# robotic-vision-lab/Edge-Informed-Contrast-Maximization

Hardware: AMD Instinct MI355X
Metric: warped-events/sec/GPU + loss+grad eval ms, 1e6 events @ 346x260 (higher is better)
Workload: dtype f32

## Files before the change

edge-informed-contrast-maximization_amd/csrc/eincm_api.hip:

```cpp
#include <hip/hip_runtime.h>
#include <hip/hip_ext.h>

#include <algorithm>
#include <chrono>
#include <cmath>
#include <cstdarg>
#include <cstdio>
#include <cstdlib>
#include <cstring>
#include <string>
#include <vector>

#include "eincm.h"
#include "eincm_kernels.hip.h"
#include "eincm_kernels_f64.hip.h"
#include "eincm_binning.hip.h"
#include "eincm_edges.hip.h"
#include "eincm_objectives.hip.h"
#include "eincm_splat_window.hip.h"
#include "eincm_canny.hip.h"
#include "eincm_preprocess.hip.h"
#include "eincm_gtflow.hip.h"
#include "eincm_dsec.hip.h"
#include "eincm_floweval.hip.h"
// ... 39 lines not shown
        if (p) { v.push_back(Block{p, bytes}); total += bytes; }
        return hipSuccess;
    }
    static bool drop(std::vector<Block>& v, size_t& total, void* p, hipError_t (*free_fn)(void*)) {
        for (size_t i = 0; i < v.size(); ++i)
            if (v[i].p == p) { (void)free_fn(p); total -= v[i].bytes; v.erase(v.begin() + i); return true; }
        return false;
    }
};

template <typename T, bool PINNED = false> struct Grow {
    T* p = nullptr;
    size_t n = 0;
};

struct Carve {
    size_t total = 0;
    size_t add(size_t bytes) { const size_t off = total; total += (bytes + 255) & ~(size_t)255; return off; }
};

struct SegList {
    int seg = 0;
    int n = 0;
    double tspan = 1.0;
    Item* d_items = nullptr;
    int32_t* d_order = nullptr;
    std::vector<Item> h_items;
    std::vector<int32_t> h_order;
    int32_t* d_win_item0 = nullptr;
    std::vector<int32_t> h_win_item0;
    Window* d_wins = nullptr;
    int32_t* d_itembase = nullptr;
    unsigned grid(int R) const { return (unsigned)(((n + NXCD - 1) / NXCD) * NXCD * R); }
};

struct WinFit {
    int cap, maxw;
    bool pal;
    bool fits;
};

struct EvalPlan {
    enum Shape { IDENTITY, TWO_DOF, GRID } shape = GRID;
    enum ThetaSrc { THETA_DEVICE, THETA_ARGS, THETA_PINNED, THETA_PIECES } theta_src = THETA_PIECES;
    int h = 0, w = 0; size_t nth = 0;
    bool want_grad = false, full_aux = false, div_grad = false;
    EvalParams ep{};
    bool obj = false; ObjGeom og{};
    int wincap = 0, winmaxw = 0, pitch_aligned = 0, wincap_a = 0, winmaxw_a = 0;
    WinFit win_2{}; bool splat_short = false;
    bool use_arg = false, use_arg_big = false;
    bool need_theta_image = false;
    bool host_asm = false;
    bool grid_tail = false;
    bool stream_stats = false, g2_from_imgrad = false;
    bool tv_proj = false, proj = false;
    bool all_r = false;
    bool events_projected = false; int nsrc = 0;
    bool zero_copy_out = false;
};

struct StagePlan {
    Geom g{};
    int64_t N = 0;
    int seg = 0, seg_s = 0, seg_2 = 0;
    bool splat_short = false;
    int pitch = 0;
    bool sort_segments = true;
    bool spread = true;
    bool host_binning = false;
    bool defer_constants = false;
    bool wide = false;
};

constexpr int SEG_SHORT = 8192;
constexpr int MIN_SEG = 64;

struct StageArgs {
    int B, R; const int64_t* n_events;
    const int16_t* const* xs; const int16_t* const* ys; const double* const* ts; const double* const* edges; const double* edge_ts;
    uint32_t flags;
};

struct StageScratch {
    std::vector<unsigned> cntmax; std::vector<double> dtmax;
    bool edge_ts_uploaded = false;
    std::vector<BinBlock> blks; std::vector<int32_t> win_blk; int32_t misc[4]; std::vector<double> mom;
    std::vector<uint32_t> sxy; std::vector<double> st; std::vector<float> ef;
    std::vector<int> ishift;
};

}

struct eincm_ctx {
    int device = 0;
    int H = 0, W = 0, maxR = 0, maxB = 0;
    int64_t maxN = 0;
    uint32_t cflags = 0;
    int seg = 0;
    int seg_s = 0;
    hipStream_t stream = nullptr;
    std::string err;
    Mem mem;

    bool staged = false;
    StagePlan stage;
    Geom g{};
    std::vector<int64_t> win_events;

    uint32_t* d_xy = nullptr;
    double* d_t = nullptr;
    uint32_t* d_xy_g = nullptr;
    double* d_t_g = nullptr;
    std::vector<int32_t> h_tilecount;
    SegList gather;
    SegList splat;
    SegList splat_sh;
    SegList gather_2;
    bool policy_evaluated = false;
    int wincap = WIN_CAP_DEFAULT;
    bool wincap_fixed = false;
    int16_t* d_raw_x = nullptr; int16_t* d_raw_y = nullptr; double* d_raw_t = nullptr;
    BinBlock* d_binblocks = nullptr; int32_t* d_win_blk = nullptr; uint32_t* d_blockhist = nullptr;
    int32_t* d_tilecount = nullptr; int32_t* d_tilebase = nullptr; int32_t* d_bin_misc = nullptr;
    bool itembase_valid = false;
    double* d_edges_raw = nullptr; double* d_edge_moments = nullptr;
    int64_t max_binblocks = 0;
    bool host_binning = false;
    int64_t max_items = 0;
    float* d_edges = nullptr;
    double* d_edge_ts = nullptr;
    unsigned long long* d_acc = nullptr;
    float* d_iwe = nullptr;
    float* d_G = nullptr;
    float* d_zero_iwe = nullptr;
    double* d_Theta = nullptr;
    double* d_theta_in = nullptr;
    long long* d_gTheta = nullptr;
    double* d_g11 = nullptr;
    double* d_dtmax = nullptr;
    unsigned* d_gmax = nullptr;
// ... 304 lines not shown
            tr[(size_t)ty * tilesX + tx] = q;
        }
    HIPCHK(c, hipMemcpyAsync(c->d_tilerng, tr.data(), tr.size() * sizeof(TileRange), hipMemcpyHostToDevice, c->stream));
    c->proj_in_gather = fits && !getenv("EINCM_NO_PROJ_IN_GATHER");
    HIPCHK(c, hipStreamSynchronize(c->stream));
    c->cur_h = h; c->cur_w = w; c->cur_method = method;
    return EINCM_OK;
}

constexpr size_t ZERO_COPY_MAX = 65536;


int win_maxw(int cap) { return std::max(40, (int)std::lround(std::sqrt((double)cap * 1.4))); }

WinFit fit_window(double vmax, double tspan, double margin, int floor_k, int pitch) {
    static const int caps[] = {2304, 3072, 4608, 6912};
    const double side = TS + margin + vmax * tspan, sd = std::ceil(side);
    const double need = pitch < 0 ? side * side : sd * sd;
    int cap = caps[3];
    for (int k = floor_k; k < 4; ++k) if (need <= caps[k]) { cap = caps[k]; break; }
    return WinFit{cap, win_maxw(cap), pitch > 0 && std::ceil(sd / 32.0) * 32.0 * sd <= (double)cap, need <= (double)caps[3]};
}

int clear_accumulators(eincm_ctx* c) {
    const size_t img = (size_t)c->H * c->W;
    HIPCHK(c, hipMemsetAsync(c->d_acc, 0, (size_t)c->maxB * c->maxR * img * sizeof(unsigned long long), c->stream));
    HIPCHK(c, hipMemsetAsync(c->d_gTheta, 0, (size_t)c->maxB * img * 2 * sizeof(long long), c->stream));
    HIPCHK(c, hipMemsetAsync(c->d_gth.p, 0, (size_t)2 * c->maxB * c->coarse_cap * sizeof(long long), c->stream));
    c->acc_dirty = false;
    return EINCM_OK;
}

void launch_theta_image(eincm_ctx* c, int h, int w, bool identity, bool use_arg, const ThetaArgBig& targ, const double* theta_dev,
                        bool with_windows) {
    const Geom& g = c->g;
    const bool ww = with_windows && c->itembase_valid;
    auto go = [&](auto kernel, const auto& ta) {
        launch_timed(c, EINCM_STAGE_THETA, kernel, dim3(g.ntiles, g.B), dim3(NT), 0, g, h, w, identity ? 1 : 0, use_arg ? 1 : 0, ta,
                     theta_dev, c->d_AH.p, c->d_AW.p, c->d_rowtap, c->d_coltap, c->d_tilerng, c->d_Theta, c->d_tmm, c->d_edge_ts,
                     c->gather.n, c->gather.d_items, ww ? c->gather.d_itembase : nullptr, c->gather.d_wins,
                     c->splat.n, c->splat.d_items, ww ? c->splat.d_itembase : nullptr, c->splat.d_wins);
    };
    if (!use_arg || (size_t)g.B * h * w * 2 <= (size_t)THETA_ARG_MID) {
        ThetaArgMid mid;
        if (use_arg) memcpy(mid.v, targ.v, (size_t)g.B * h * w * 2 * sizeof(double));
        go(k_theta<ThetaArgMid>, mid);
// ... 31 lines not shown
    {
        StageTimer t(c, EINCM_STAGE_THETA, two_dof ? !P.need_theta_image : c->itembase_valid);
        const SegList &ga = c->gather, &sp = c->splat;
        const int nwin_threads = (ga.n + sp.n) * g.R;
        if (two_dof) {
            if (theta_host) c->last_theta11.assign(theta_host, theta_host + (size_t)g.B * 2); else c->last_theta11.clear();
            c->Theta_valid = false;
            if (P.need_theta_image) launch_theta_image(c, P.h, P.w, false, P.use_arg_big, targ_big, theta_dev, false);
            if (!P.host_asm)
                launch_timed(c, EINCM_STAGE_THETA, k_theta_const, dim3((std::max(g.B * g.ntiles, nwin_threads) + NT - 1) / NT), dim3(NT), 0, g,
                                   P.use_arg ? 1 : 0, targ, theta_dev, c->d_tmm, c->d_edge_ts, ga.n, ga.d_items, ga.d_wins,
                                   sp.n, sp.d_items, sp.d_wins);
        } else {
            launch_theta_image(c, P.h, P.w, P.shape == EvalPlan::IDENTITY, P.use_arg_big, targ_big, theta_dev, true);
            if (nwin_threads > 0 && !c->itembase_valid)
                hipLaunchKernelGGL(k_windows, dim3((nwin_threads + NT - 1) / NT), dim3(NT), 0, c->stream, g, c->d_tmm, c->d_edge_ts,
                                   ga.n, ga.d_items, ga.d_wins, sp.n, sp.d_items, sp.d_wins);
        }
    }
    {
        StageTimer t(c, EINCM_STAGE_SPLAT, true);
        c->acc_dirty = true;
        if (c->splat.n > 0) {
            const SegList& L = P.splat_short ? c->splat_sh : c->splat;
            const size_t theta_tile = two_dof ? 0 : TS * TS * sizeof(double2);
            const int use_arg = P.use_arg ? 1 : 0;
            if (c->splat_rad != 1) {
                Geom gs = g;
                gs.wincap = std::min(g.wincap, two_dof ? SW_CAP_CONST : SW_CAP_TILE);
                gs.winmaxw = win_maxw(gs.wincap);
                auto go = [&](auto kernel) {
                    launch_timed(c, EINCM_STAGE_SPLAT, kernel, dim3(L.grid(g.R)), dim3(NT), (size_t)gs.wincap * sizeof(unsigned long long) + theta_tile,
                                 gs, L.n, L.d_items, c->d_xy, c->d_t, c->d_Theta, c->d_tmm, c->d_edge_ts, c->d_acc, L.d_order, use_arg, theta_dev, targ);
                };
                if (two_dof) c->splat_rad == 0 ? go(k_splat_r<THETA_CONST, 0>) : c->splat_rad == 2 ? go(k_splat_r<THETA_CONST, 2>) : go(k_splat_r<THETA_CONST, 3>);
                else         c->splat_rad == 0 ? go(k_splat_r<THETA_TILE, 0>) : c->splat_rad == 2 ? go(k_splat_r<THETA_TILE, 2>) : go(k_splat_r<THETA_TILE, 3>);
            } else {
                auto go = [&](auto kernel) {
                    launch_timed(c, EINCM_STAGE_SPLAT, kernel, dim3(L.grid(g.R)), dim3(512), (size_t)g.wincap * sizeof(float) + theta_tile, g, L.n,
                                 L.d_items, c->d_xy, c->d_t, c->d_Theta, c->d_edge_ts, c->splat.d_wins, c->d_acc, L.d_order, use_arg, theta_dev, targ);
                };
                two_dof ? go(k_splat<THETA_CONST, 512>) : go(k_splat<THETA_TILE, 512>);
            }
        }
    }
    HIPCHK(c, hipGetLastError());
    c->pend.theta_dev = theta_dev; c->pend.targ = targ;
// ... 232 lines not shown
    if (c->fp64) return P;
    const size_t nall = (size_t)g.B * P.nth;

    static const bool no_big_arg = getenv("EINCM_NO_BIG_THETA_ARG") != nullptr;
    P.use_arg = !c->theta_dev_in && !identity && nall <= (size_t)THETA_ARG_MAX;
    P.use_arg_big = !c->theta_dev_in && !identity && nall <= (size_t)THETA_ARG_BIG && !no_big_arg;
    P.theta_src = c->theta_dev_in ? EvalPlan::THETA_DEVICE
                : (P.use_arg_big && (P.use_arg || !two_dof)) ? EvalPlan::THETA_ARGS
                : nall <= ZERO_COPY_MAX ? EvalPlan::THETA_PINNED : EvalPlan::THETA_PIECES;
    P.need_theta_image = !two_dof || ep.want_tv || c->theta_dev_in;

    P.wincap = g.wincap; P.winmaxw = g.winmaxw; P.wincap_a = g.wincap_a; P.winmaxw_a = g.winmaxw_a;
    P.pitch_aligned = c->stage.pitch != 0 ? 1 : 0;
    P.win_2 = WinFit{c->wincap, win_maxw(c->wincap), c->stage.pitch >= 2, true};
    if (!c->wincap_fixed) {
        double vmax = 0.0;
        const size_t stride = nall > 8192 ? nall / 8192 : 1;
        if (c->theta_dev_in) vmax = (c->vmax_hint >= 0.0 && std::isfinite(c->vmax_hint)) ? c->vmax_hint : 1e9;
        else if (stride == 1) { for (size_t i = 0; i < nall; ++i) { const double a = std::fabs(theta_host[i]); vmax = std::max(vmax, a <= 1.7e308 ? a : 0.0); } }
        else for (size_t i = 0; i < nall; i += stride) { const double a = std::fabs(theta_host[i]); if (a > vmax && std::isfinite(a)) vmax = a; }
        const double margin = 2.0 * (c->splat_rad + 1);
        const int floor_s = two_dof ? 2 : 0, pitch_s = c->stage.pitch != 0 ? 1 : 0;
        WinFit s = fit_window(vmax, c->splat.tspan, margin, floor_s, pitch_s);
        P.splat_short = two_dof && c->splat_sh.n > 0 && !s.fits;
        if (P.splat_short) s = fit_window(vmax, c->splat_sh.tspan, margin, floor_s, pitch_s);
        P.wincap = s.cap; P.winmaxw = s.maxw; P.pitch_aligned = s.pal ? 1 : 0;
        const WinFit a = fit_window(vmax, c->gather.tspan, margin, 2, -1);
        P.wincap_a = a.cap; P.winmaxw_a = a.maxw;
        P.win_2 = fit_window(vmax, c->gather_2.tspan, margin, 2, c->stage.pitch >= 2 ? 1 : 0);
    }

    static const bool no_host_asm = getenv("EINCM_NO_HOST_ASM") != nullptr;
    const bool tail_ok = c->splat_rad == 1 && P.shape == EvalPlan::GRID && c->proj_in_gather && c->itembase_valid && nall <= ZERO_COPY_MAX &&
                         !c->theta_dev_in;
    P.host_asm = want_grad && ((two_dof && !ep.want_tv) || tail_ok) && !ep.want_div && !P.full_aux && !no_host_asm && !c->device_results &&
                 !c->theta_dev_in;
    P.grid_tail = P.host_asm && P.shape == EvalPlan::GRID;
    P.g2_from_imgrad = want_grad && ep.contrast_kind == EINCM_CONTRAST_GRAD_MAG && !P.obj;
    P.stream_stats = P.host_asm || (P.g2_from_imgrad && g.ntiles >= NSPART) || P.obj;
    P.tv_proj = ep.use_tv_grad && P.shape == EvalPlan::GRID && c->proj_in_gather;
    P.proj = want_grad && P.shape == EvalPlan::GRID && c->proj_in_gather && c->splat_rad == 1;
    static const int all_r_env = getenv("EINCM_GATHER_ALL_R") ? atoi(getenv("EINCM_GATHER_ALL_R")) : -1;
    P.all_r = P.proj && (all_r_env >= 0 ? all_r_env != 0 : c->gather.n >= 700);
    P.events_projected = two_dof || P.proj;
    P.nsrc = (!want_grad || identity) ? 0 : (P.events_projected ? 0 : 1) + ((ep.use_tv_grad && !P.tv_proj) ? 1 : 0);
    P.zero_copy_out = !c->device_results && !c->theta_dev_in && !identity && nall <= ZERO_COPY_MAX;
    return P;
}

void scan_theta(eincm_ctx* c, const double* theta_host, size_t nth) {
    c->theta_nan.assign((size_t)c->g.B, 0);
    for (int b = 0; b < c->g.B; ++b) {
// ... 147 lines not shown
                           c->d_wc, c->d_objc.p, c->d_gdiv.p, c->d_dgparts.p, c->d_G, c->d_gmax, c->h_ovals.p, 0);
    }
    if (want_grad) {
        {
            StageTimer t(c, EINCM_STAGE_IMGRAD, !P.div_grad && !P.obj);
            if (P.div_grad)
                hipLaunchKernelGGL(k_divgrad, dim3(g.ntiles, g.R, g.B), dim3(NT), 0, c->stream, g, c->d_iwe, c->d_parts,
                                   c->d_gdiv.p, c->d_dgparts.p);
            if (P.obj) {
                const ObjGeom& og = P.og;
                hipLaunchKernelGGL(k_obj_parts, dim3(og.ncells, g.R, g.B), dim3(NT), 0, c->stream, g, og, c->d_iwe, 1, c->d_edges, c->d_oparts.p);
                hipLaunchKernelGGL(k_obj_grad, dim3(n_imwg, g.R, g.B), dim3(IG_NT), 0, c->stream, g, ep, og, c->d_iwe, c->d_edges, c->d_oparts.p,
                                   c->d_wc, c->d_objc.p, c->d_gdiv.p, c->d_dgparts.p, c->d_G, c->d_gmax, c->h_ovals.p, 1);
            } else {
                launch_timed(c, EINCM_STAGE_IMGRAD, k_imgrad, dim3(n_imwg, g.R, g.B), dim3(IG_NT), 0, g, ep, c->d_iwe, c->d_edges,
                                   c->d_parts, c->d_wc, c->d_gdiv.p, c->d_dgparts.p, host_asm ? c->h_g2 : c->d_g2parts, c->d_G, c->d_gmax,
                                   host_asm ? c->h_img : nullptr, host_asm ? 1 : 0);
            }
        }
        {
            StageTimer t(c, EINCM_STAGE_GATHER, true);
            constexpr int NT_TILE = 512;
            if (c->gather.n > 0) {
                const SegList& L = two_dof ? c->gather_2 : c->gather;
                const uint32_t* xy_g = two_dof ? c->d_xy : c->d_xy_g;
                const double* t_g = two_dof ? c->d_t : c->d_t_g;
                Geom gg = g;
                if (two_dof) { gg.pitch_aligned = P.win_2.pal ? 1 : 0; gg.wincap_a = P.win_2.cap; gg.winmaxw_a = P.win_2.maxw; }
                const dim3 grid(L.grid(P.all_r ? 1 : g.R));
                const size_t lds = gg.wincap_a * sizeof(float) + (two_dof ? 0 : TS * TS * 2 * sizeof(double) + TS * TS * sizeof(double2));
                double* g11 = host_asm ? c->h_g11 : c->d_g11;
                const int use_arg = P.use_arg ? 1 : 0;
                if (c->splat_rad != 1) {
                    auto go = [&](auto kernel) {
                        launch_timed(c, EINCM_STAGE_GATHER, kernel, grid, dim3(NT), lds, gg, L.n, L.d_items, xy_g, t_g, c->d_Theta, c->d_tmm,
                                     c->d_edge_ts, c->d_G, c->d_gTheta, g11, c->d_wc, c->d_gmax, c->stage.wide ? 1 : 0, use_arg, c->pend.theta_dev,
                                     c->pend.targ);
                    };
                    if (two_dof) c->splat_rad == 0 ? go(k_gather_r<THETA_CONST, 0>) : c->splat_rad == 2 ? go(k_gather_r<THETA_CONST, 2>) : go(k_gather_r<THETA_CONST, 3>);
                    else         c->splat_rad == 0 ? go(k_gather_r<THETA_TILE, 0>) : c->splat_rad == 2 ? go(k_gather_r<THETA_TILE, 2>) : go(k_gather_r<THETA_TILE, 3>);
                } else {
                    auto go = [&](auto kernel, int nthreads) {
                        launch_timed(c, EINCM_STAGE_GATHER, kernel, grid, dim3(nthreads), lds, gg, L.n, L.d_items, xy_g, t_g, c->d_Theta,
                                     c->d_edge_ts, c->d_G, c->gather.d_wins, c->d_gTheta, g11, c->d_wc, c->d_gmax, L.d_order, use_arg,
                                     c->pend.theta_dev, c->pend.targ, P.h, P.w, c->d_AH.p, c->d_AW.p, c->d_tilerng, c->d_gth.p, (int)c->coarse_cap,
                                     P.grid_tail ? 1 : 0, c->d_gticket, c->gather.d_win_item0, c->h_grad,
                                     (P.grid_tail && ep.use_tv_grad) ? ep.gamma : 0.0, c->d_tvparts, c->d_gth.p + (size_t)c->maxB * c->coarse_cap);
                    };
                    if (two_dof)      go(k_gather<THETA_CONST, 0, NT, 0>, NT);
                    else if (P.all_r) c->stage.wide ? go(k_gather<THETA_TILE, 1, NT_TILE, 1, 1>, NT_TILE) : go(k_gather<THETA_TILE, 0, NT_TILE, 1, 1>, NT_TILE);
                    else if (c->stage.wide) P.proj ? go(k_gather<THETA_TILE, 1, NT_TILE, 1>, NT_TILE) : go(k_gather<THETA_TILE, 1, NT_TILE, 0>, NT_TILE);
                    else              P.proj ? go(k_gather<THETA_TILE, 0, NT_TILE, 1>, NT_TILE) : go(k_gather<THETA_TILE, 0, NT_TILE, 0>, NT_TILE);
                }
            }
        }
        if (P.nsrc > 0) {
            StageTimer t(c, EINCM_STAGE_PROJECT, true);
            launch_timed(c, EINCM_STAGE_PROJECT, k_project, dim3(g.ntiles, g.B, P.nsrc), dim3(NT), 0, g, P.h, P.w,
                               (int)c->coarse_cap, P.events_projected ? 1 : 0, c->stage.wide ? 1 : 0, c->d_AH.p, c->d_AW.p, c->d_rowtap, c->d_coltap, c->d_gTheta, c->d_tvg,
                               c->d_wc, c->d_gmax, c->d_gth.p, c->d_gth.p + (size_t)c->maxB * c->coarse_cap);
        }
    }
    if (!host_asm) {
        StageTimer t(c, EINCM_STAGE_FINAL, !(want_grad && identity));
        launch_timed(c, EINCM_STAGE_FINAL, k_final, dim3(g.B), dim3(FT), 0, g, ep, c->d_parts, c->d_divparts, c->d_tvparts,
                           c->d_tmm, c->d_wc, P.g2_from_imgrad ? c->d_g2parts : nullptr, c->d_gth.p, c->d_gth.p + (size_t)c->maxB * c->coarse_cap, (int)c->coarse_cap,
                           c->d_g11, c->gather_2.d_win_item0, c->gather_2.n, c->d_gmax,
                           P.zero_copy_out ? c->h_outs : c->d_outs, P.zero_copy_out ? c->h_grad : c->d_grad, want_grad ? 1 : 0);
        if (want_grad && identity) {
            hipLaunchKernelGGL(k_final_dense, dim3(256, g.B), dim3(NT), 0, c->stream, g, ep.use_tv_grad, c->stage.wide ? 1 : 0, c->d_gTheta,
                               c->d_tvg, c->d_wc, c->d_gmax, c->d_outs, c->d_grad);
        }
    }
    HIPCHK(c, hipGetLastError());
    c->n_pieces = 0;
    c->pend.copy_mode = (P.zero_copy_out || host_asm) ? 0 : 1;
    if (c->pend.copy_mode && !c->device_results) { const int rcc = enqueue_result_copies(c); if (rcc) return rcc; c->pend.copy_mode = 0; }
    if (timing && c->ring_size == 1) { (void)hipEventRecord(c->ev[c->ring_cur][EINCM_N_STAGES][1], c->stream); c->ev_used[c->ring_cur][EINCM_N_STAGES] = true; }
    c->pend.launched = true;
    c->acc_dirty = false;
    return EINCM_OK;
}

void host_assemble(eincm_ctx* c) {
    const Geom& g = c->g;
    const EvalPlan& P = c->pend.plan;
    const EvalParams& ep = P.ep;
    const double HW = (double)g.H * (double)g.W;
    for (int b = 0; b < g.B; ++b) {
        const WinConst& wc = c->h_wc[b];
// ... 1 lines not shown
        memset(&o, 0, sizeof o);
        if (b < 64 && !((g.wmask >> b) & 1ull)) continue;
        double sum_rel_con = 0.0, sum_rel_corr = 0.0;
        for (int r = 0; r < g.R; ++r) {
            const double* q = c->h_img + ((size_t)b * g.R + r) * IMGSCAL_N;
            ImgScal s{};
            s.m = q[0]; s.M = q[1]; s.D = q[2]; s.cm = q[3]; s.cM = q[4]; s.sI = q[5]; s.sII = q[6]; s.sEI = q[7];
            double g2 = 0.0;
            const int nwg = (g.nig + IG_NT / 64 - 1) / (IG_NT / 64);
            const double* g2p = c->h_g2 + ((size_t)b * g.R + r) * nwg;
            for (int i = 0; i < nwg; ++i) g2 += g2p[i];
            const double mse = mse_from_moments(s, wc.sE[r], wc.sEE[r], HW);
            const double mean = s.sI / HW;
            const double var = s.sII / HW - mean * mean;
            const double cgm = g2 / HW;
            const double con = (ep.contrast_kind == 1) ? var : cgm;
            const double c0 = (ep.contrast_kind == 1) ? wc.c0_var : wc.c0_gradmag;
            o.corr[r] = -mse; o.contrast_gm[r] = cgm; o.var[r] = var; o.div[r] = NAN;
            sum_rel_con += wc.mrw[r] * con / (c0 + EPSN);
            sum_rel_corr += wc.mrw[r] * (-mse) / (wc.zc[r] + EPSN);
        }
        assemble_window(ep, g.R, sum_rel_con, sum_rel_corr, NAN, window_tv(c, ep, b), c->theta_nan[b] != 0, true, o);
        if (P.shape == EvalPlan::TWO_DOF) {
            const int lo = c->gather_2.h_win_item0[b], hi = c->gather_2.h_win_item0[b + 1];
            const double* p = c->h_g11 + (size_t)lo * g.R * 2;
            const size_t n = (size_t)(hi - lo) * g.R;
            double ax[4] = {0.0, 0.0, 0.0, 0.0}, ay[4] = {0.0, 0.0, 0.0, 0.0};
            size_t k = 0;
            for (; k + 4 <= n; k += 4) {
                ax[0] += p[2 * k]; ay[0] += p[2 * k + 1]; ax[1] += p[2 * k + 2]; ay[1] += p[2 * k + 3];
                ax[2] += p[2 * k + 4]; ay[2] += p[2 * k + 5]; ax[3] += p[2 * k + 6]; ay[3] += p[2 * k + 7];
            }
            for (; k < n; ++k) { ax[0] += p[2 * k]; ay[0] += p[2 * k + 1]; }
            c->h_grad[(size_t)b * 2] = (ax[0] + ax[1]) + (ax[2] + ax[3]); c->h_grad[(size_t)b * 2 + 1] = (ay[0] + ay[1]) + (ay[2] + ay[3]);
        } else if (c->win_events[b] == 0) {
            for (size_t i = 0; i < P.nth; ++i) c->h_grad[(size_t)b * P.nth + i] = 0.0;
        }
    }
}

int eval_end_collect(eincm_ctx* c, double* value, double* grad, eincm_aux* aux) {
    if (!c->pend.active || !c->pend.launched) return fail(c, EINCM_ERR_STATE, "no evaluation in flight");
    const Geom& g = c->g;
    const bool want_grad = c->pend.plan.want_grad;
    const size_t nth = c->pend.plan.nth;
    if (c->pend.copy_mode) { const int rcc = enqueue_result_copies(c); c->pend.copy_mode = 0; if (rcc) { (void)hipStreamSynchronize(c->stream); c->pend.active = false; c->pend.launched = false; return rcc; } }
    bool piece_bad = false;
// ... 192 lines not shown
    c->fp64 = (flags & EINCM_CF_FP64) != 0;
    c->device = device; c->H = H; c->W = W; c->maxR = max_refs; c->maxB = max_windows; c->maxN = max_events_total;
    c->cflags = flags;
    auto bail = [&](const char* what, hipError_t err) -> eincm_ctx* {
        fail(nullptr, EINCM_ERR_HIP, "eincm_create: %s failed: %s", what, hipGetErrorString(err));
        free_all(c);
        delete c;
        return nullptr;
    };
#define TRY(expr) do { hipError_t e2_ = (expr); if (e2_ != hipSuccess) return bail(#expr, e2_); } while (0)
    TRY(hipSetDevice(device));
    TRY(hipStreamCreateWithFlags(&c->stream, hipStreamNonBlocking));
    const int tilesX = (W + TS - 1) / TS, tilesY = (H + TS - 1) / TS, ntiles = tilesX * tilesY;
    const size_t B = max_windows, R = max_refs, img = (size_t)H * W;
    if (const char* s = getenv("EINCM_SEG")) { int v = atoi(s); if (v >= MIN_SEG && v <= MAX_SEG) c->seg = v; }
    if (const char* s = getenv("EINCM_SEG_SPLAT")) { int v = atoi(s); if (v >= MIN_SEG && v <= MAX_CHUNK) c->seg_s = v; }
    if (const char* s = getenv("EINCM_WINCAP")) { int v = atoi(s); if (v >= 1024 && v <= 6912) { c->wincap = (v / 4) * 4; c->wincap_fixed = true; } }
    c->host_binning = (ntiles > BIN_MAX_TILES) || (getenv("EINCM_HOST_BINNING") != nullptr);
    c->max_items = (int64_t)B * ntiles + max_events_total / MIN_SEG + 1;
    TRY(c->mem.alloc_dev(c->d_xy, (size_t)max_events_total));
    TRY(c->mem.alloc_dev(c->d_t, (size_t)max_events_total));
    TRY(c->mem.alloc_dev(c->d_xy_g, (size_t)max_events_total));
    TRY(c->mem.alloc_dev(c->d_t_g, (size_t)max_events_total));
    for (SegList* L : {&c->gather, &c->splat, &c->splat_sh, &c->gather_2}) {
        TRY(c->mem.alloc_dev(L->d_items, (size_t)c->max_items));
        TRY(c->mem.alloc_dev(L->d_order, (size_t)c->max_items));
    }
    for (SegList* L : {&c->gather, &c->gather_2}) TRY(c->mem.alloc_dev(L->d_win_item0, B + 1));
    for (SegList* L : {&c->gather, &c->splat}) {
        TRY(c->mem.alloc_dev(L->d_wins, (size_t)c->max_items * max_refs));
        if (!c->host_binning) TRY(c->mem.alloc_dev(L->d_itembase, B * ntiles));
    }
    TRY(c->mem.alloc_dev(c->d_raw_x, (size_t)max_events_total));
    TRY(c->mem.alloc_dev(c->d_raw_y, (size_t)max_events_total));
    TRY(c->mem.alloc_dev(c->d_raw_t, (size_t)max_events_total));
    if (!c->host_binning) {
        c->max_binblocks = max_events_total / BIN_CHUNK + (int64_t)B + 1;
        TRY(c->mem.alloc_dev(c->d_binblocks, (size_t)c->max_binblocks));
        TRY(c->mem.alloc_dev(c->d_win_blk, B + 1));
        TRY(c->mem.alloc_dev(c->d_blockhist, (size_t)c->max_binblocks * ntiles));
        TRY(c->mem.alloc_dev(c->d_tilecount, B * ntiles));
        TRY(c->mem.alloc_dev(c->d_tilebase, B * ntiles));
        TRY(c->mem.alloc_dev(c->d_bin_misc, (size_t)8));
        TRY(c->mem.alloc_dev(c->d_edges_raw, B * R * img));
        TRY(c->mem.alloc_dev(c->d_edge_moments, B * R * EDGE_PARTS * EDGE_MOM));
    }
    TRY(c->mem.alloc_dev(c->d_edges, B * R * img));
// ... 163 lines not shown
}

static StagePlan plan_staging(const eincm_ctx* c, const StageArgs& a) {
    StagePlan P;
    const int H = c->H, W = c->W, n_windows = a.B, n_refs = a.R;
    Geom& g = P.g;
    g.H = H; g.W = W; g.R = n_refs; g.B = n_windows;
    g.tilesX = (W + TS - 1) / TS; g.tilesY = (H + TS - 1) / TS; g.ntiles = g.tilesX * g.tilesY;
    g.igx = (W + IG_COLS - 1) / IG_COLS; g.nig = g.igx * ((H + IG_ROWS - 1) / IG_ROWS);
    g.pstride = std::max(g.ntiles, NSPART);
    g.gmax_n = g.R * g.nig;
    g.wincap = c->wincap; g.winmaxw = win_maxw(c->wincap);
    g.wincap_a = g.wincap; g.winmaxw_a = g.winmaxw;
    for (int b = 0; b < n_windows; ++b) P.N += a.n_events[b];
    const int64_t N = P.N;

    const double x_wg = ((double)N / 8192.0 + 0.5 * n_windows * g.ntiles) * n_refs;
    const double per_tile = (double)N / ((double)n_windows * g.ntiles);
    P.seg = c->seg > 0 ? c->seg : 16384;
    P.seg_2 = (x_wg >= 4000.0 && per_tile < 16384.0) ? 16384 : (x_wg < 1000.0 ? 4096 : 8192);
    if (const char* e = getenv("EINCM_SEG_2DOF")) { const int v = atoi(e); if (v >= MIN_SEG && v <= MAX_SEG) P.seg_2 = v; }
    P.seg_s = c->seg_s > 0 ? c->seg_s : (x_wg >= 3000.0 && per_tile < 16384.0 ? 16384 : (x_wg >= 400.0 ? 8192 : 4096));
    P.splat_short = P.seg_s > SEG_SHORT && N > 0;
    P.pitch = (x_wg >= 3000.0 && per_tile < 16384.0) ? 1 : 0;
    if (const char* e = getenv("EINCM_PITCH_ALIGNED")) P.pitch = std::max(0, std::min(2, atoi(e)));
    g.pitch_aligned = P.pitch;
    P.sort_segments = getenv("EINCM_NO_SEGSORT") == nullptr;
    P.spread = getenv("EINCM_NO_SPREAD") == nullptr;
    P.host_binning = c->host_binning;
    P.defer_constants = (a.flags & EINCM_SW_DEFER_CONSTANTS) != 0;
    P.wide = std::any_of(a.n_events, a.n_events + n_windows, [&](int64_t n) { return n * (int64_t)n_refs < 4096; });
    return P;
}

static int refuse_event(eincm_ctx* c, const StageArgs& a, int b, int64_t i, bool bad_xy) {
    if (!bad_xy) return fail(c, EINCM_ERR_ARG, "event %lld of window %d has a non-finite timestamp", (long long)i, b);
    return fail(c, EINCM_ERR_ARG, "event %lld of window %d at (x=%d, y=%d) outside the %dx%d sensor", (long long)i, b, (int)a.xs[b][i],
                (int)a.ys[b][i], c->H, c->W);
}
static int refuse_event_at(eincm_ctx* c, const StageArgs& a, int64_t e, bool bad_xy) {
    int b = 0;
    while (b < a.B - 1 && e >= a.n_events[b]) { e -= a.n_events[b]; ++b; }
    return refuse_event(c, a, b, e, bad_xy);
}

static int upload_raw_events(eincm_ctx* c, const StageArgs& a) {
// ... 145 lines not shown
    sc.ef.resize((size_t)a.B * a.R * img);
    for (int b = 0; b < a.B; ++b) {
        WinConst& wc = c->h_wc[b];
        for (int r = 0; r < a.R; ++r) {
            const double* e = a.edges[b] + (size_t)r * img;
            float* o = sc.ef.data() + ((size_t)b * a.R + r) * img;
            double s = 0.0, ss = 0.0, mx = 0.0;
            for (size_t i = 0; i < img; ++i) { const float f = (float)e[i]; o[i] = f; s += (double)f; ss += (double)f * (double)f; mx = std::max(mx, std::fabs((double)f)); }
            wc.sE[r] = s; wc.sEE[r] = ss; wc.eabs[r] = mx;
        }
    }
    if (P.N > 0) {
        HIPCHK(c, hipMemcpyAsync(c->d_xy, sc.sxy.data(), (size_t)P.N * sizeof(uint32_t), hipMemcpyHostToDevice, c->stream));
        HIPCHK(c, hipMemcpyAsync(c->d_t, sc.st.data(), (size_t)P.N * sizeof(double), hipMemcpyHostToDevice, c->stream));
        if ((rc = upload_raw_events(c, a))) return rc;
    }
    if ((rc = build_list(c, c->gather, P.seg, true, g.ntiles, c->d_t, P.N))) return rc;
    if ((rc = copy_for_gather(c))) return rc;
    if ((rc = build_list(c, c->splat, P.seg_s, true, g.ntiles, c->d_t, P.N))) return rc;
    HIPCHK(c, hipMemcpyAsync(c->d_edges, sc.ef.data(), sc.ef.size() * sizeof(float), hipMemcpyHostToDevice, c->stream));
    return EINCM_OK;
}

static int finish_lists(eincm_ctx* c, const StageArgs& a, StageScratch& sc) {
    const StagePlan& P = c->stage;
    const Geom& g = P.g;
    int rc = EINCM_OK;
    if (!sc.edge_ts_uploaded)
        HIPCHK(c, hipMemcpyAsync(c->d_edge_ts, a.edge_ts, (size_t)a.B * a.R * sizeof(double), hipMemcpyHostToDevice, c->stream));
    HIPCHK(c, hipMemsetAsync(c->d_mask, 0, (size_t)a.B * g.H * g.W, c->stream));
    if ((rc = build_list(c, c->gather_2, P.seg_2, true, g.ntiles, c->d_t, P.N))) return rc;
    c->splat_sh.n = 0;
    if (P.splat_short && (rc = build_list(c, c->splat_sh, SEG_SHORT, true, g.ntiles, c->d_t, P.N))) return rc;
    if (c->gather.n > 0 && !P.host_binning) {
        HIPCHK(c, hipMemsetAsync(c->d_cntmax, 0, (size_t)a.B * sizeof(unsigned), c->stream));
        hipLaunchKernelGGL(k_tile_counts, dim3(g.ntiles, a.B), dim3(NT), 0, c->stream, g, c->d_tilebase, c->d_tilecount, c->d_xy,
                           c->d_mask, c->d_cntmax);
        HIPCHK(c, hipGetLastError());
        HIPCHK(c, hipMemcpyAsync(sc.cntmax.data(), c->d_cntmax, (size_t)a.B * sizeof(unsigned), hipMemcpyDeviceToHost, c->stream));
    }
    HIPCHK(c, hipStreamSynchronize(c->stream));
    c->policy_evaluated = false;
    c->g = g;
    c->itembase_valid = !P.host_binning && c->gather.n > 0 && c->splat.n > 0;
    c->win_events.assign(a.n_events, a.n_events + a.B);
    if (c->gather.n > 0 && P.host_binning) {
        hipLaunchKernelGGL(k_mask, dim3(std::min(c->gather.n, 2048)), dim3(NT), 0, c->stream, g, c->gather.d_items, c->gather.n, c->d_xy, c->d_mask);
        HIPCHK(c, hipGetLastError());
    }
    return EINCM_OK;
}

static int stage_fp64(eincm_ctx* c, const StageArgs& a, StageScratch& sc) {
    const size_t img = (size_t)c->H * c->W;
    for (int b = 0; b < a.B; ++b) sc.ishift.push_back(f64_ishift(a.n_events[b]));
    HIPCHK(c, hipMemcpyAsync(c->f64.ishift, sc.ishift.data(), sc.ishift.size() * sizeof(int), hipMemcpyHostToDevice, c->stream));
// ... 1188 lines not shown
    if (reset) { c->sum_t = eincm_timings{}; c->sum_n = 0; }
    return EINCM_OK;
}

int eincm_get_host_profile(eincm_ctx* c, double* us, int64_t* n_evals, int reset) {
    if (!c || !us || !n_evals) return EINCM_ERR_ARG;
    for (int i = 0; i < EINCM_N_HOST_PHASES; ++i) us[i] = c->hp_us[i];
    *n_evals = c->hp_n;
    if (reset) { for (double& v : c->hp_us) v = 0.0; c->hp_n = 0; }
    return EINCM_OK;
}

int eincm_get_memory(eincm_ctx* c, int64_t out[4]) {
    if (!c || !out) return EINCM_ERR_ARG;
    out[0] = (int64_t)c->mem.dev_bytes; out[1] = (int64_t)c->mem.pinned_bytes;
    out[2] = (int64_t)(c->mem.dev.size() + c->mem.pinned.size()); out[3] = (int64_t)c->scratch.n;
    return EINCM_OK;
}

int eincm_get_launch_policy(eincm_ctx* c, double* out) {
    if (!c || !out) return EINCM_ERR_ARG;
    const StagePlan& S = c->stage;
    out[EINCM_LP_SEG_GATHER] = S.seg; out[EINCM_LP_SEG_SPLAT] = S.seg_s; out[EINCM_LP_SEG_GATHER_2DOF] = S.seg_2;
    out[EINCM_LP_SEG_SPLAT_SHORT] = S.splat_short ? SEG_SHORT : 0; out[EINCM_LP_PITCH_POLICY] = S.pitch;
    out[EINCM_LP_SPAN_SPLAT] = c->splat.tspan; out[EINCM_LP_SPAN_GATHER] = c->gather.tspan; out[EINCM_LP_SPAN_GATHER_2DOF] = c->gather_2.tspan;
    const bool evaluated = c->policy_evaluated;
    const EvalPlan& P = c->pend.plan;
    out[EINCM_LP_CAP_SPLAT] = evaluated ? P.wincap : 0; out[EINCM_LP_CAP_GATHER] = evaluated ? P.wincap_a : 0;
    out[EINCM_LP_CAP_GATHER_2DOF] = evaluated ? P.win_2.cap : 0;
    out[EINCM_LP_PITCH_ALIGNED] = evaluated ? ((P.pitch_aligned ? 1 : 0) | (P.win_2.pal ? 2 : 0)) : 0;
    out[EINCM_LP_SPLAT_SHORT] = evaluated && P.splat_short ? 1 : 0;
    return EINCM_OK;
}

int eincm_set_timed_kernels(eincm_ctx* c, int splat, int gather) {
    if (!c) return EINCM_ERR_ARG;
    if (!(c->cflags & EINCM_CF_TIMING_DOMINANT)) return fail(c, EINCM_ERR_STATE, "context was created without EINCM_CF_TIMING_DOMINANT");
    if (c->pend.active) return fail(c, EINCM_ERR_STATE, "an evaluation is in flight");
    c->time_splat = splat != 0; c->time_gather = gather != 0;
    return EINCM_OK;
}

int eincm_set_timing_period(eincm_ctx* c, int period) {
    if (!c) return EINCM_ERR_ARG;
    if (!(c->cflags & EINCM_CF_TIMING_DOMINANT)) return fail(c, EINCM_ERR_STATE, "context was created without EINCM_CF_TIMING_DOMINANT");
    if (c->pend.active) return fail(c, EINCM_ERR_STATE, "an evaluation is in flight");
    if (period < 1) return fail(c, EINCM_ERR_ARG, "period %d", period);
    c->time_period = period; c->time_counter = 0;
    return EINCM_OK;
}

int eincm_get_timings(eincm_ctx* c, eincm_timings* t) {
    if (!c || !t) return EINCM_ERR_ARG;
    if (!(c->cflags & (EINCM_CF_TIMING | EINCM_CF_TIMING_DOMINANT)))
// ... 205 lines not shown
```

edge-informed-contrast-maximization_amd/engine.py:

```python
import ctypes as C
from typing import NamedTuple

import numpy as np

from . import _lib as L


class EincmError(RuntimeError):
    def __init__(self, code, msg):
        super().__init__(f'eincm error {code}: {msg}')
        self.code = code


class NonFiniteLoss(EincmError):
    pass


def _dp(a):
    return a.ctypes.data_as(C.POINTER(C.c_double))


def as_int16_coords(a, what='coordinates'):
    a = np.asarray(a)
    if a.dtype == np.int16:
# ... 909 lines not shown
        wx = np.empty((self.R, n), dtype=np.float64)
        wy = np.empty((self.R, n), dtype=np.float64)
        self._check(self._lib.eincm_get_warped_events(self._ctx, int(window), _dp(wx), _dp(wy)))
        return wx, wy

    def scaled_theta(self):
        a = np.empty((self.B, self.H, self.W, 2), dtype=np.float64)
        self._check(self._lib.eincm_get_scaled_theta(self._ctx, _dp(a)))
        return a

    def timings_total(self, reset=False):
        t = L.Timings(); n = C.c_int64(0)
        self._check(self._lib.eincm_get_timings_total(self._ctx, C.byref(t), C.byref(n), 1 if reset else 0))
        d = {name: float(t.ms[i]) for i, name in enumerate(L.STAGE_NAMES)}
        d['total'] = float(t.total_ms)
        return d, int(n.value)

    def host_profile(self, reset=False):
        us = (C.c_double * 4)(); n = C.c_int64(0)
        self._check(self._lib.eincm_get_host_profile(self._ctx, us, C.byref(n), 1 if reset else 0))
        return dict(zip(('begin', 'launch', 'wait', 'collect'), (float(v) for v in us))), int(n.value)

    LAUNCH_POLICY_NAMES = ('seg_gather', 'seg_splat', 'seg_gather_2dof', 'seg_splat_short', 'pitch_policy', 'span_splat', 'span_gather',
                           'span_gather_2dof', 'cap_splat', 'cap_gather', 'cap_gather_2dof', 'pitch_aligned', 'splat_short')

    def launch_policy(self):
        out = (C.c_double * len(self.LAUNCH_POLICY_NAMES))()
        self._check(self._lib.eincm_get_launch_policy(self._ctx, out))
        return dict(zip(self.LAUNCH_POLICY_NAMES, (float(v) for v in out)))

    def memory(self):
        out = (C.c_int64 * 4)()
        self._check(self._lib.eincm_get_memory(self._ctx, out))
        return Memory(*(int(v) for v in out))

    def set_timed_kernels(self, splat=True, gather=True):
        self._check(self._lib.eincm_set_timed_kernels(self._ctx, 1 if splat else 0, 1 if gather else 0))

    def set_timing_period(self, period):
        self._check(self._lib.eincm_set_timing_period(self._ctx, int(period)))

    def timings(self):
        t = L.Timings()
        self._check(self._lib.eincm_get_timings(self._ctx, C.byref(t)))
        d = {n: float(t.ms[i]) for i, n in enumerate(L.STAGE_NAMES)}
        d['total'] = float(t.total_ms)
        return d
# ... 84 lines not shown
```

include/eincm.h:

```cpp
#ifndef EINCM_H
#define EINCM_H

#include <stdint.h>

#ifdef __cplusplus
extern "C" {
#endif

#define EINCM_ABI_VERSION 6

#define EINCM_OK               0
#define EINCM_ERR_ARG         -1
#define EINCM_ERR_HIP         -2
#define EINCM_ERR_STATE       -3
#define EINCM_ERR_NONFINITE   -4
#define EINCM_ERR_UNSUPPORTED -5

#define EINCM_CONTRAST_GRAD_MAG 0
#define EINCM_CONTRAST_VARIANCE 1
#define EINCM_CONTRAST_ADAPTIVE_GRAD_MAG 2
#define EINCM_CONTRAST_ADAPTIVE_VARIANCE 3

#define EINCM_CORRELATION_MSE            0
#define EINCM_CORRELATION_ADAPTIVE_MSE   1
// ... 127 lines not shown
int eincm_get_timings(eincm_ctx* ctx, eincm_timings* t);
int eincm_set_timed_kernels(eincm_ctx* ctx, int splat, int gather);
int eincm_set_timing_period(eincm_ctx* ctx, int period);

#define EINCM_HP_BEGIN 0
#define EINCM_HP_LAUNCH 1
#define EINCM_HP_WAIT 2
#define EINCM_HP_COLLECT 3
#define EINCM_N_HOST_PHASES 4
int eincm_get_host_profile(eincm_ctx* ctx, double* us , int64_t* n_evals, int reset);
#define EINCM_LP_SEG_GATHER 0
#define EINCM_LP_SEG_SPLAT 1
#define EINCM_LP_SEG_GATHER_2DOF 2
#define EINCM_LP_SEG_SPLAT_SHORT 3
#define EINCM_LP_PITCH_POLICY 4
#define EINCM_LP_SPAN_SPLAT 5
#define EINCM_LP_SPAN_GATHER 6
#define EINCM_LP_SPAN_GATHER_2DOF 7
#define EINCM_LP_CAP_SPLAT 8
#define EINCM_LP_CAP_GATHER 9
#define EINCM_LP_CAP_GATHER_2DOF 10
#define EINCM_LP_PITCH_ALIGNED 11
#define EINCM_LP_SPLAT_SHORT 12
#define EINCM_N_LAUNCH_POLICY 13
int eincm_get_launch_policy(eincm_ctx* ctx, double* out );

int eincm_get_memory(eincm_ctx* ctx, int64_t out[4]);
int eincm_get_timings_total(eincm_ctx* ctx, eincm_timings* sum, int64_t* n_evals, int reset);

int eincm_loss_grad_device(eincm_ctx* ctx, const double* theta_dev, int h, int w, const eincm_params* p, double theta_abs_max,
                           double* value, double* grad_dev, eincm_aux* aux);

int eincm_set_device_results(eincm_ctx* ctx, int on);
int eincm_finish_launch(eincm_ctx* ctx);
int eincm_grad_device_ptr(eincm_ctx* ctx, void** dptr, int64_t* n_doubles);
int eincm_finish_collect(eincm_ctx* ctx, double* value, double* grad, eincm_aux* aux);

int eincm_forward_iwe(eincm_ctx* ctx, const double* theta, int h, int w, const eincm_params* p, int want_grad);
int eincm_finish_loss_grad(eincm_ctx* ctx, double* value, double* grad, eincm_aux* aux);
int eincm_finish_constants(eincm_ctx* ctx);
int eincm_iwe_device_ptr(eincm_ctx* ctx, void** dptr, int64_t* n_words);
int eincm_mask_device_ptr(eincm_ctx* ctx, void** dptr, int64_t* n_bytes);

#define EINCM_EDT_EXPONENTIAL 0
#define EINCM_EDT_LINEAR 1
#define EINCM_EDT_LINEAR_BOUND 2
#define EINCM_EDT_LOGARITHMIC 3
// ... 97 lines not shown
```

Measured before the change: 177.8 billion.

## Build a family of shorter segment lists and pick the longest that fits per eval

Replaces the single short splat list with a family of progressively halved segment lists for both the splat and 2-DOF gather passes, built at staging time. Each evaluation picks the longest segment list whose warped window, computed from the current per-window velocity, fits the shared-memory window cap. The aim is to keep the fast windowed path with fewer, longer work items when velocities allow, and fall back to shorter segments only when needed. The cost is extra list building and device memory at staging, plus host-side selection logic on every eval.

```diff
diff --git a/edge-informed-contrast-maximization_amd/csrc/eincm_api.hip b/edge-informed-contrast-maximization_amd/csrc/eincm_api.hip
--- a/edge-informed-contrast-maximization_amd/csrc/eincm_api.hip
+++ b/edge-informed-contrast-maximization_amd/csrc/eincm_api.hip
@@ -85,6 +85,7 @@
 struct SegList {
     int seg = 0;
     int n = 0;
+    int64_t cap = 0;
     double tspan = 1.0;
     Item* d_items = nullptr;
     int32_t* d_order = nullptr;
@@ -111,7 +112,8 @@
     EvalParams ep{};
     bool obj = false; ObjGeom og{};
     int wincap = 0, winmaxw = 0, pitch_aligned = 0, wincap_a = 0, winmaxw_a = 0;
-    WinFit win_2{}; bool splat_short = false;
+    WinFit win_2{};
+    int list_s = 0, list_2 = 0; bool splat_short = false;
     bool use_arg = false, use_arg_big = false;
     bool need_theta_image = false;
     bool host_asm = false;
@@ -128,6 +130,8 @@
     int64_t N = 0;
     int seg = 0, seg_s = 0, seg_2 = 0;
     bool splat_short = false;
+    bool family = true;
+    int force_seg = 0;
     int pitch = 0;
     bool sort_segments = true;
     bool spread = true;
@@ -137,6 +141,7 @@
 };
 
 constexpr int SEG_SHORT = 8192;
+constexpr int SEG_FAMILY_MIN = 2048;
 constexpr int MIN_SEG = 64;
 
 struct StageArgs {
@@ -178,8 +183,9 @@
     std::vector<int32_t> h_tilecount;
     SegList gather;
     SegList splat;
-    SegList splat_sh;
+    std::vector<SegList> splat_fam; int n_fam_s = 0;
     SegList gather_2;
+    std::vector<SegList> gather2_fam; int n_fam_2 = 0;
     bool policy_evaluated = false;
     int wincap = WIN_CAP_DEFAULT;
     bool wincap_fixed = false;
@@ -530,6 +536,29 @@
     return WinFit{cap, win_maxw(cap), pitch > 0 && std::ceil(sd / 32.0) * 32.0 * sd <= (double)cap, need <= (double)caps[3]};
 }
 
+const SegList& family_list(const SegList& base, const std::vector<SegList>& fam, int k) { return k > 0 ? fam[(size_t)k - 1] : base; }
+
+bool has_short_list(const eincm_ctx* c) { return c->stage.splat_short && c->n_fam_s > 0 && c->splat_fam[0].seg == SEG_SHORT; }
+
+int pick_list(const eincm_ctx* c, const SegList& base, const std::vector<SegList>& fam, int n_fam, const double* theta11, double vmax, double margin) {
+    constexpr int CAP = 6912;
+    const int maxw = win_maxw(CAP);
+    const Geom& g = c->g;
+    auto mag = [](double v) { const double a = std::fabs(v); return a <= 1.7e308 ? a : 0.0; };
+    for (int k = 0; k <= n_fam; ++k) {
+        const double tspan = family_list(base, fam, k).tspan;
+        bool fits = true;
+        for (int b = 0; b < g.B && fits; ++b) {
+            if (b < 64 && !((g.wmask >> b) & 1ull)) continue;
+            const double ww = std::ceil(TS + margin + (theta11 ? mag(theta11[2 * b]) : vmax) * tspan);
+            const double wh = std::ceil(TS + margin + (theta11 ? mag(theta11[2 * b + 1]) : vmax) * tspan);
+            fits = ww * wh <= (double)CAP && ww <= (double)maxw;
+        }
+        if (fits) return k;
+    }
+    return n_fam;
+}
+
 int clear_accumulators(eincm_ctx* c) {
     const size_t img = (size_t)c->H * c->W;
     HIPCHK(c, hipMemsetAsync(c->d_acc, 0, (size_t)c->maxB * c->maxR * img * sizeof(unsigned long long), c->stream));
@@ -607,7 +636,7 @@
         StageTimer t(c, EINCM_STAGE_SPLAT, true);
         c->acc_dirty = true;
         if (c->splat.n > 0) {
-            const SegList& L = P.splat_short ? c->splat_sh : c->splat;
+            const SegList& L = family_list(c->splat, c->splat_fam, P.list_s);
             const size_t theta_tile = two_dof ? 0 : TS * TS * sizeof(double2);
             const int use_arg = P.use_arg ? 1 : 0;
             if (c->splat_rad != 1) {
@@ -886,12 +915,30 @@
         const double margin = 2.0 * (c->splat_rad + 1);
         const int floor_s = two_dof ? 2 : 0, pitch_s = c->stage.pitch != 0 ? 1 : 0;
         WinFit s = fit_window(vmax, c->splat.tspan, margin, floor_s, pitch_s);
-        P.splat_short = two_dof && c->splat_sh.n > 0 && !s.fits;
-        if (P.splat_short) s = fit_window(vmax, c->splat_sh.tspan, margin, floor_s, pitch_s);
+        if (two_dof) {
+            const bool known = !c->theta_dev_in || vmax < 1e9;
+            if (c->stage.family && known) {
+                const double* th11 = c->theta_dev_in ? nullptr : theta_host;
+                P.list_s = pick_list(c, c->splat, c->splat_fam, c->n_fam_s, th11, vmax, margin);
+                P.list_2 = pick_list(c, c->gather_2, c->gather2_fam, c->n_fam_2, th11, vmax, margin);
+            } else {
+                P.list_s = (has_short_list(c) && !s.fits) ? 1 : 0;
+            }
+            if (c->stage.force_seg > 0) {
+                auto forced = [&](const SegList& base, const std::vector<SegList>& fam, int n_fam) {
+                    for (int k = 0; k <= n_fam; ++k) if (family_list(base, fam, k).seg <= c->stage.force_seg) return k;
+                    return n_fam;
+                };
+                P.list_s = forced(c->splat, c->splat_fam, c->n_fam_s);
+                P.list_2 = forced(c->gather_2, c->gather2_fam, c->n_fam_2);
+            }
+        }
+        P.splat_short = P.list_s > 0;
+        if (P.splat_short) s = fit_window(vmax, family_list(c->splat, c->splat_fam, P.list_s).tspan, margin, floor_s, pitch_s);
         P.wincap = s.cap; P.winmaxw = s.maxw; P.pitch_aligned = s.pal ? 1 : 0;
         const WinFit a = fit_window(vmax, c->gather.tspan, margin, 2, -1);
         P.wincap_a = a.cap; P.winmaxw_a = a.maxw;
-        P.win_2 = fit_window(vmax, c->gather_2.tspan, margin, 2, c->stage.pitch >= 2 ? 1 : 0);
+        P.win_2 = fit_window(vmax, family_list(c->gather_2, c->gather2_fam, P.list_2).tspan, margin, 2, c->stage.pitch >= 2 ? 1 : 0);
     }
 
     static const bool no_host_asm = getenv("EINCM_NO_HOST_ASM") != nullptr;
@@ -1085,7 +1132,7 @@
             StageTimer t(c, EINCM_STAGE_GATHER, true);
             constexpr int NT_TILE = 512;
             if (c->gather.n > 0) {
-                const SegList& L = two_dof ? c->gather_2 : c->gather;
+                const SegList& L = two_dof ? family_list(c->gather_2, c->gather2_fam, P.list_2) : c->gather;
                 const uint32_t* xy_g = two_dof ? c->d_xy : c->d_xy_g;
                 const double* t_g = two_dof ? c->d_t : c->d_t_g;
                 Geom gg = g;
@@ -1126,9 +1173,10 @@
     }
     if (!host_asm) {
         StageTimer t(c, EINCM_STAGE_FINAL, !(want_grad && identity));
+        const SegList& L2 = family_list(c->gather_2, c->gather2_fam, P.list_2);
         launch_timed(c, EINCM_STAGE_FINAL, k_final, dim3(g.B), dim3(FT), 0, g, ep, c->d_parts, c->d_divparts, c->d_tvparts,
                            c->d_tmm, c->d_wc, P.g2_from_imgrad ? c->d_g2parts : nullptr, c->d_gth.p, c->d_gth.p + (size_t)c->maxB * c->coarse_cap, (int)c->coarse_cap,
-                           c->d_g11, c->gather_2.d_win_item0, c->gather_2.n, c->d_gmax,
+                           c->d_g11, L2.d_win_item0, L2.n, c->d_gmax,
                            P.zero_copy_out ? c->h_outs : c->d_outs, P.zero_copy_out ? c->h_grad : c->d_grad, want_grad ? 1 : 0);
         if (want_grad && identity) {
             hipLaunchKernelGGL(k_final_dense, dim3(256, g.B), dim3(NT), 0, c->stream, g, ep.use_tv_grad, c->stage.wide ? 1 : 0, c->d_gTheta,
@@ -1176,7 +1224,8 @@
         }
         assemble_window(ep, g.R, sum_rel_con, sum_rel_corr, NAN, window_tv(c, ep, b), c->theta_nan[b] != 0, true, o);
         if (P.shape == EvalPlan::TWO_DOF) {
-            const int lo = c->gather_2.h_win_item0[b], hi = c->gather_2.h_win_item0[b + 1];
+            const SegList& L2 = family_list(c->gather_2, c->gather2_fam, P.list_2);
+            const int lo = L2.h_win_item0[b], hi = L2.h_win_item0[b + 1];
             const double* p = c->h_g11 + (size_t)lo * g.R * 2;
             const size_t n = (size_t)(hi - lo) * g.R;
             double ax[4] = {0.0, 0.0, 0.0, 0.0}, ay[4] = {0.0, 0.0, 0.0, 0.0};
@@ -1415,7 +1464,8 @@
     TRY(c->mem.alloc_dev(c->d_t, (size_t)max_events_total));
     TRY(c->mem.alloc_dev(c->d_xy_g, (size_t)max_events_total));
     TRY(c->mem.alloc_dev(c->d_t_g, (size_t)max_events_total));
-    for (SegList* L : {&c->gather, &c->splat, &c->splat_sh, &c->gather_2}) {
+    for (int len = MAX_SEG; len >= 2 * SEG_FAMILY_MIN; len /= 2) { c->splat_fam.emplace_back(); c->gather2_fam.emplace_back(); }
+    for (SegList* L : {&c->gather, &c->splat, &c->gather_2}) {
         TRY(c->mem.alloc_dev(L->d_items, (size_t)c->max_items));
         TRY(c->mem.alloc_dev(L->d_order, (size_t)c->max_items));
     }
@@ -1625,6 +1675,8 @@
     if (const char* e = getenv("EINCM_SEG_2DOF")) { const int v = atoi(e); if (v >= MIN_SEG && v <= MAX_SEG) P.seg_2 = v; }
     P.seg_s = c->seg_s > 0 ? c->seg_s : (x_wg >= 3000.0 && per_tile < 16384.0 ? 16384 : (x_wg >= 400.0 ? 8192 : 4096));
     P.splat_short = P.seg_s > SEG_SHORT && N > 0;
+    P.family = getenv("EINCM_NO_SEG_FAMILY") == nullptr;
+    if (const char* e = getenv("EINCM_SEG_FORCE")) { const int v = atoi(e); if (v >= MIN_SEG && v <= MAX_SEG) P.force_seg = v; }
     P.pitch = (x_wg >= 3000.0 && per_tile < 16384.0) ? 1 : 0;
     if (const char* e = getenv("EINCM_PITCH_ALIGNED")) P.pitch = std::max(0, std::min(2, atoi(e)));
     g.pitch_aligned = P.pitch;
@@ -1816,6 +1868,40 @@
     return EINCM_OK;
 }
 
+static int shorter_seg(int len) { const int h = len / 2; return (h >= SEG_FAMILY_MIN && h % 256 == 0 && len % 2 == 0) ? h : 0; }
+
+static int ensure_list(eincm_ctx* c, SegList& L, int seg, bool win_item0) {
+    const int64_t ntiles = (int64_t)((c->W + TS - 1) / TS) * ((c->H + TS - 1) / TS);
+    const int64_t need = (int64_t)c->maxB * ntiles + c->maxN / seg + 1;
+    if (win_item0 && !L.d_win_item0) HIPCHK(c, c->mem.alloc_dev(L.d_win_item0, (size_t)c->maxB + 1));
+    if (L.cap >= need) return EINCM_OK;
+    HIPCHK(c, hipStreamSynchronize(c->stream));
+    c->mem.release(L.d_items); c->mem.release(L.d_order);
+    L.d_items = nullptr; L.d_order = nullptr; L.cap = 0;
+    HIPCHK(c, c->mem.alloc_dev(L.d_items, (size_t)need));
+    HIPCHK(c, c->mem.alloc_dev(L.d_order, (size_t)need));
+    L.cap = need;
+    return EINCM_OK;
+}
+
+static int build_family(eincm_ctx* c, const SegList& base, std::vector<SegList>& fam, int& n_fam, int first, bool always, bool win_item0) {
+    const StagePlan& P = c->stage;
+    n_fam = 0;
+    int n_longer = base.n;
+    for (int len = first; len > 0 && (size_t)n_fam < fam.size(); len = always ? 0 : shorter_seg(len)) {
+        int64_t n = 0;
+        for (const int32_t cnt : c->h_tilecount) n += (cnt + len - 1) / len;
+        if (!always && n <= n_longer) continue;
+        SegList& L = fam[(size_t)n_fam];
+        int rc = ensure_list(c, L, len, win_item0);
+        if (!rc) rc = build_list(c, L, len, true, P.g.ntiles, c->d_t, P.N);
+        if (rc) return rc;
+        ++n_fam;
+        n_longer = (int)n;
+    }
+    return EINCM_OK;
+}
+
 static int finish_lists(eincm_ctx* c, const StageArgs& a, StageScratch& sc) {
     const StagePlan& P = c->stage;
     const Geom& g = P.g;
@@ -1824,8 +1910,9 @@
         HIPCHK(c, hipMemcpyAsync(c->d_edge_ts, a.edge_ts, (size_t)a.B * a.R * sizeof(double), hipMemcpyHostToDevice, c->stream));
     HIPCHK(c, hipMemsetAsync(c->d_mask, 0, (size_t)a.B * g.H * g.W, c->stream));
     if ((rc = build_list(c, c->gather_2, P.seg_2, true, g.ntiles, c->d_t, P.N))) return rc;
-    c->splat_sh.n = 0;
-    if (P.splat_short && (rc = build_list(c, c->splat_sh, SEG_SHORT, true, g.ntiles, c->d_t, P.N))) return rc;
+    const int first_s = P.splat_short ? SEG_SHORT : shorter_seg(P.seg_s);
+    if ((rc = build_family(c, c->splat, c->splat_fam, c->n_fam_s, P.family ? first_s : (P.splat_short ? SEG_SHORT : 0), !P.family, false))) return rc;
+    if ((rc = build_family(c, c->gather_2, c->gather2_fam, c->n_fam_2, P.family ? shorter_seg(P.seg_2) : 0, false, true))) return rc;
     if (c->gather.n > 0 && !P.host_binning) {
         HIPCHK(c, hipMemsetAsync(c->d_cntmax, 0, (size_t)a.B * sizeof(unsigned), c->stream));
         hipLaunchKernelGGL(k_tile_counts, dim3(g.ntiles, a.B), dim3(NT), 0, c->stream, g, c->d_tilebase, c->d_tilecount, c->d_xy,
@@ -3060,7 +3147,7 @@
     if (!c || !out) return EINCM_ERR_ARG;
     const StagePlan& S = c->stage;
     out[EINCM_LP_SEG_GATHER] = S.seg; out[EINCM_LP_SEG_SPLAT] = S.seg_s; out[EINCM_LP_SEG_GATHER_2DOF] = S.seg_2;
-    out[EINCM_LP_SEG_SPLAT_SHORT] = S.splat_short ? SEG_SHORT : 0; out[EINCM_LP_PITCH_POLICY] = S.pitch;
+    out[EINCM_LP_SEG_SPLAT_SHORT] = has_short_list(c) ? SEG_SHORT : 0; out[EINCM_LP_PITCH_POLICY] = S.pitch;
     out[EINCM_LP_SPAN_SPLAT] = c->splat.tspan; out[EINCM_LP_SPAN_GATHER] = c->gather.tspan; out[EINCM_LP_SPAN_GATHER_2DOF] = c->gather_2.tspan;
     const bool evaluated = c->policy_evaluated;
     const EvalPlan& P = c->pend.plan;
@@ -3068,6 +3155,10 @@
     out[EINCM_LP_CAP_GATHER_2DOF] = evaluated ? P.win_2.cap : 0;
     out[EINCM_LP_PITCH_ALIGNED] = evaluated ? ((P.pitch_aligned ? 1 : 0) | (P.win_2.pal ? 2 : 0)) : 0;
     out[EINCM_LP_SPLAT_SHORT] = evaluated && P.splat_short ? 1 : 0;
+    const bool two_dof = evaluated && P.shape == EvalPlan::TWO_DOF;
+    out[EINCM_LP_WALKED_SPLAT] = evaluated ? family_list(c->splat, c->splat_fam, P.list_s).seg : 0;
+    out[EINCM_LP_WALKED_GATHER_2DOF] = two_dof ? family_list(c->gather_2, c->gather2_fam, P.list_2).seg : 0;
+    out[EINCM_LP_LISTS_SPLAT] = c->staged ? 1 + c->n_fam_s : 0; out[EINCM_LP_LISTS_GATHER_2DOF] = c->staged ? 1 + c->n_fam_2 : 0;
     return EINCM_OK;
 }
 
diff --git a/edge-informed-contrast-maximization_amd/engine.py b/edge-informed-contrast-maximization_amd/engine.py
--- a/edge-informed-contrast-maximization_amd/engine.py
+++ b/edge-informed-contrast-maximization_amd/engine.py
@@ -955,7 +955,8 @@
         return dict(zip(('begin', 'launch', 'wait', 'collect'), (float(v) for v in us))), int(n.value)
 
     LAUNCH_POLICY_NAMES = ('seg_gather', 'seg_splat', 'seg_gather_2dof', 'seg_splat_short', 'pitch_policy', 'span_splat', 'span_gather',
-                           'span_gather_2dof', 'cap_splat', 'cap_gather', 'cap_gather_2dof', 'pitch_aligned', 'splat_short')
+                           'span_gather_2dof', 'cap_splat', 'cap_gather', 'cap_gather_2dof', 'pitch_aligned', 'splat_short', 'walked_splat',
+                           'walked_gather_2dof', 'lists_splat', 'lists_gather_2dof')
 
     def launch_policy(self):
         out = (C.c_double * len(self.LAUNCH_POLICY_NAMES))()
diff --git a/include/eincm.h b/include/eincm.h
--- a/include/eincm.h
+++ b/include/eincm.h
@@ -173,7 +173,11 @@
 #define EINCM_LP_CAP_GATHER_2DOF 10
 #define EINCM_LP_PITCH_ALIGNED 11
 #define EINCM_LP_SPLAT_SHORT 12
-#define EINCM_N_LAUNCH_POLICY 13
+#define EINCM_LP_WALKED_SPLAT 13
+#define EINCM_LP_WALKED_GATHER_2DOF 14
+#define EINCM_LP_LISTS_SPLAT 15
+#define EINCM_LP_LISTS_GATHER_2DOF 16
+#define EINCM_N_LAUNCH_POLICY 17
 int eincm_get_launch_policy(eincm_ctx* ctx, double* out );
 
 int eincm_get_memory(eincm_ctx* ctx, int64_t out[4]);
```

Result: no change. 177.4 billion (-0.3%).
